# JMUWRobotics/3DTK

Hardware: AMD Instinct MI355X
Metric: NN correspondences/sec (1M-vs-1M pairwise ICP, full iteration) (higher is better)
Workload: dtype f64; 1 GPU; configs[1]: synthetic 1000000-vs-1000000 uniform pair, point-to-point ICP -a 1 -d 25 -b 20, 1xMI355X; points=1000000, bucket=20, minimizer=QUAT

## Files before the change

3dtk_amd/csrc/kernels.hip:

```cpp
#include <atomic>
#include <cstdio>
#include <vector>
#include <algorithm>
#include <hip/hip_runtime.h>
#include <type_traits>

#include <cmath>
#include <cstdio>
#include <cstdlib>
#include <cstring>

#include "kernels.h"
#include "lane_stack.h"
#ifdef TDTK_LAB
#include "loop_dev.h"
#endif

namespace tdtk {

#define WAVE 64
#define LAZY_MAX 8

__device__ __forceinline__ void dev_xf3(const Mat4& A, double x, double y, double z, double& ox,
                                        double& oy, double& oz)
// ... 125 lines not shown
  typedef uint32_t raw __attribute__((ext_vector_type(sizeof(V) / 4)));
  typedef const raw __attribute__((address_space(1))) * gp;
  const raw r = *(gp)(base + off);
  V v;
  __builtin_memcpy(&v, &r, sizeof v);
  return v;
}
template <class V>
__device__ __forceinline__ void gstore(char* base, const uint32_t off, const V v)
{
  typedef uint32_t raw __attribute__((ext_vector_type(sizeof(V) / 4)));
  typedef raw __attribute__((address_space(1))) * gp;
  raw r;
  __builtin_memcpy(&r, &v, sizeof v);
  *(gp)(base + off) = r;
}
#define TDTK_PIN_BATCH3(a, b, c) asm volatile("" : "+v"(a), "+v"(b), "+v"(c))

#define TDTK_PIN_V64(x) asm volatile("" : "+v"(x))
#define TDTK_PIN_S64(x) asm volatile("" : "+s"(x))
#define TDTK_PIN_S32(x) asm volatile("" : "+s"(x))
#define TDTK_PIN_SF(x) asm volatile("" : "+s"(x))
#define TDTK_PIN_VF(x) asm volatile("" : "+v"(x))

struct BoxF32 {
  float qx, qy, qz;
  float delta;
  float thi, tlo;
  float ec;
  float pthr;
  float qs, pthr16;
  __device__ __forceinline__ void set_query(const double x, const double y, const double z, const float absmax)
  {
    qx = (float)x; qy = (float)y; qz = (float)z;
    qs = 0.f;
    const float qm = fmaxf(fmaxf(fabsf(qx), fabsf(qy)), fabsf(qz));
    delta = 3.0e-7f * (qm + 2.0f * absmax) + 1.0e-30f;
    ec = 1.05e-7f * (qm + absmax) + 1.0e-30f;
    const float probe = fabsf(qx) + fabsf(qy) + fabsf(qz);
    if (!(probe <= 3.0e38f)) { delta = __builtin_nanf(""); ec = delta; }
  }
  __device__ __forceinline__ float reject_from(const float R) const
  {
    const float w = (R * 1.000001f + ec) * 1.000001f;
    const float t = w * w * 1.000001f;
    return (t <= 1.0e37f) ? t : __builtin_nanf("");
// ... 879 lines not shown
#pragma unroll
  for (int off = 32; off > 0; off >>= 1) t += __shfl_down(t, off, WAVE);
  return t;
}

template <int BLOCK, int SD, int GS = 8, bool FUSE = false, bool LOOP = false>
__global__ void __launch_bounds__(BLOCK) k_search_g8(const SearchArgs a_by_value)
{
  (void)a_by_value;
  search_g8_body<BLOCK, SD, GS, FUSE, LOOP>(kernarg_block<SearchArgs>(), blockIdx.x, gridDim.x);
}
template <int BLOCK, int SD, int GS>
__global__ void __launch_bounds__(BLOCK) k_search_g8_multi(const SearchArgs* __restrict__ args, const uint32_t* __restrict__ base,
                                                           int nbatch)
{
  int l = 0;
  while (l + 1 < nbatch && blockIdx.x >= base[l + 1]) ++l;
  l = __builtin_amdgcn_readfirstlane(l);
  const uint32_t b0 = base[l], b1 = base[l + 1];
  search_g8_body<BLOCK, SD, GS>(args[l], blockIdx.x - b0, b1 - b0);
}

#define WTRACE_MAX 32768u
#ifdef TDTK_LAB
__device__ unsigned long long g_wtrace[3 * WTRACE_MAX];
#else
__device__ unsigned long long g_wtrace[3];
#endif

struct RefillCfg {
  static constexpr int BLOCK = 128, SD = 4;
  static constexpr int THRESH = 16, WPS = 4;
  static constexpr bool COUNT = false;
  static constexpr int FUSE = 0;
  static constexpr bool ORDER = true; static constexpr int ORD_MAX = 256;
  static constexpr bool LAZY = false;
  static constexpr bool DEFER = false;
  static constexpr bool DYN = false, FAT = false, SHARE = false, PIPE = false;
  static constexpr int PTS = 4, PROBE = 0, TOP = 0;
};
template <class CFG>
__device__ __forceinline__ void search_refill_body(const SearchArgs& a, const uint32_t bid, const uint32_t nb)
{
  constexpr int BLOCK = CFG::BLOCK, SD = CFG::SD, THRESH = CFG::THRESH, FUSE = CFG::FUSE, PTS = CFG::PTS, PROBE = CFG::PROBE, ORD_MAX = CFG::ORD_MAX, TOP = CFG::TOP;
  constexpr bool COUNT = CFG::COUNT, DYN = CFG::DYN, ORDER = CFG::ORDER, FAT = CFG::FAT, LAZY = CFG::LAZY, SHARE = CFG::SHARE, PIPE = CFG::PIPE, DEFER = CFG::DEFER;
  __shared__ uint4 lds_stk[SD][BLOCK];
  __shared__ uint4 lds_top[TOP > 0 ? 3 * TOP : 1];
  uint32_t top_n = 0;
  if constexpr (TOP > 0) {
    top_n = min((uint32_t)TOP, a.T.n_hot);
    const uint4* __restrict__ h16 = reinterpret_cast<const uint4*>(a.T.hot);
    for (uint32_t k = threadIdx.x; k < 3u * top_n; k += BLOCK) lds_top[k] = h16[k];
    __syncthreads();
  }

  const size_t gl = (size_t)bid * BLOCK + threadIdx.x;
  const unsigned lane = threadIdx.x & (WAVE - 1);
  if (kLab && a.trace && lane == 0) {
    const uint32_t wid0 = bid * (BLOCK / WAVE) + threadIdx.x / WAVE;
    if (wid0 < WTRACE_MAX) g_wtrace[3 * wid0] = wall_clock64();
  }
  __shared__ double lds_mv[LAZY ? LAZY_MAX * 16 : 1];
  if constexpr (LAZY) {
    if (a.nmoves) {
      const double* gm = reinterpret_cast<const double*>(a.moves);
      for (int k = threadIdx.x; k < a.nmoves * 16; k += BLOCK) lds_mv[k] = gm[k];
      __syncthreads();
    }
  }
  LaneStackQ<BLOCK, SD> st;
  st.l_e = &lds_stk[0][threadIdx.x];
  st.g_m2 = a.ovf_m2; st.g_ref = a.ovf_ref; st.gcol = gl;
  st.gstride = (size_t)nb * BLOCK;
  st.sp = 0;

  const TreeDev& T = a.T;
  const double4* __restrict__ nodes = reinterpret_cast<const double4*>(T.nodes);
  const double4* __restrict__ pts = reinterpret_cast<const double4*>(T.pts);
  const LeafEntry* const t_leaf_tab = T.leaf_tab;
  const uint32_t t_cb = T.cb, t_cmask = T.cmask;
  int* const a_kpos = a.kpos;
  double* const a_d2 = a.d2;
  unsigned char* const a_cost = a.cost;
  const char* const t_grp = reinterpret_cast<const char*>(T.grp);
  const char* const t_fat = reinterpret_cast<const char*>(T.fat);
  typedef typename std::conditional<(ORD_MAX > 256), unsigned short, unsigned char>::type ord_t;
  __shared__ ord_t lds_order[ORDER ? BLOCK / WAVE : 1][ORDER ? ORD_MAX : 4];
  ord_t* const my_order = lds_order[ORDER ? threadIdx.x / WAVE : 0];
  constexpr bool CERT = DEFER && BUCKET_Q16 && !LAZY && !FAT && !PIPE && TOP == 0 && PROBE == 0 && FUSE == 3 && !DYN && !SHARE && ORDER;
  static_assert(!CERT || (ORD_MAX >= CERT_MAX_SLAB && ORD_MAX / WAVE <= 32), "a slab with certificates is one ordered piece");
  bool ordered = false;
  size_t piece0 = 0;
  uint32_t walkbits = 0xFFFFFFFFu, n_listed = 0;
  auto order_piece = [&](size_t p0, size_t p1) {
    ordered = false;
    piece0 = p0;
    if (!ORDER || !a.use_cost || !a.cost || p1 <= p0 || p1 - p0 > (size_t)ORD_MAX) return;
    const uint32_t cntp = (uint32_t)(p1 - p0);
    int cls[ORD_MAX / WAVE];
    unsigned cvv[ORD_MAX / WAVE];
    unsigned mn = 255u, mx = 0u;
#pragma unroll
    for (int r = 0; r < ORD_MAX / WAVE; r++) {
      const uint32_t o = (uint32_t)r * WAVE + lane;
      const bool w = o < cntp && (!CERT || ((walkbits >> r) & 1u) != 0u);
      cvv[r] = w ? (unsigned)a.cost[p0 + o] : 0u;
      if (w) { mn = min(mn, cvv[r]); mx = max(mx, cvv[r]); }
    }
#pragma unroll
    for (int off = 32; off > 0; off >>= 1) {
      mn = min(mn, (unsigned)__shfl_xor((int)mn, off, WAVE));
      mx = max(mx, (unsigned)__shfl_xor((int)mx, off, WAVE));
    }
    const unsigned span = (mx > mn) ? mx - mn + 1u : 1u;
#pragma unroll
    for (int r = 0; r < ORD_MAX / WAVE; r++) {
      const uint32_t o = (uint32_t)r * WAVE + lane;
      const bool w = o < cntp && (!CERT || ((walkbits >> r) & 1u) != 0u);
      cls[r] = w ? (int)min(((cvv[r] - mn) * 8u) / span, 7u) : -1;
    }
    uint32_t base = 0;
    for (int k = 7; k >= 0; k--) {
#pragma unroll
      for (int r = 0; r < ORD_MAX / WAVE; r++) {
        if ((uint32_t)r * WAVE >= cntp) continue;
        const unsigned long long m = __ballot(cls[r] == k);
        if (cls[r] == k) my_order[base + (uint32_t)__popcll(m & ((1ull << lane) - 1ull))] = (ord_t)(r * WAVE + lane);
        base += (uint32_t)__popcll(m);
      }
    }
    __builtin_amdgcn_fence(__ATOMIC_SEQ_CST, "wavefront");
    __builtin_amdgcn_wave_barrier();
    ordered = true;
    n_listed = base;
  };
  const bool certw = CERT && a.cert != nullptr;
  __shared__ uint4 lds_cert[CERT ? BLOCK : 1];
  float* const my_slot = reinterpret_cast<float*>(&lds_cert[CERT ? threadIdx.x : 0]);
  unsigned c_skh = 0, c_skn = 0, c_walk = 0;
  auto cert_sweep = [&](size_t p0, size_t p1) {
    walkbits = 0u;
    const uint32_t q0 = (uint32_t)p0, cntp = (uint32_t)(p1 - p0);
    for (uint32_t r = 0; r < (uint32_t)(ORD_MAX / WAVE); r++) {
      const uint32_t o = r * WAVE + lane;
      if (o >= cntp) continue;
      const uint32_t q = q0 + o, q8 = q << 3, q4 = q << 2;
      const SearchArgs* ap = &a;
      asm volatile("" : "+s"(ap));
      const int kp = gload<int>(reinterpret_cast<const char*>(a_kpos), q4);
      const float Lq = ap->cert_use ? gload<float>(reinterpret_cast<const char*>(ap->cert), q4) : 0.f;
      const double ox = gload<double>(reinterpret_cast<const char*>(ap->x), q8), oy = gload<double>(reinterpret_cast<const char*>(ap->y), q8),
                   oz = gload<double>(reinterpret_cast<const char*>(ap->z), q8);
      double tx = ox, ty = oy, tz = oz;
      if (ap->has_pending) {
        dev_xf3_inplace(ap->pending, tx, ty, tz);
        gstore<double>(reinterpret_cast<char*>(ap->x), q8, tx); gstore<double>(reinterpret_cast<char*>(ap->y), q8, ty);
        gstore<double>(reinterpret_cast<char*>(ap->z), q8, tz);
        if (ap->nx) {
          double px = ap->nx[q], py = ap->ny[q], pz = ap->nz[q];
          dev_xf3normal(ap->pending, px, py, pz);
          ap->nx[q] = px; ap->ny[q] = py; ap->nz[q] = pz;
        }
      }
      const SearchArgs* ap2 = &a;
      asm volatile("" : "+s"(ap2), "+v"(tx));
      double ax = ox, ay = oy, az = oz, bxq = tx, byq = ty, bzq = tz;
      if (ap2->has_inv) { dev_xf3(ap2->inv, ox, oy, oz, ax, ay, az); dev_xf3(ap2->inv, tx, ty, tz, bxq, byq, bzq); }
      const double ex = bxq - ax, ey = byq - ay, ez = bzq - az;
      const float mv = __builtin_amdgcn_sqrtf((float)(ex * ex + ey * ey + ez * ez) * 1.000001f) * 1.000001f;
      const float qm = fmaxf(fmaxf(fabsf((float)bxq), fabsf((float)byq)), fabsf((float)bzq));
      const SearchArgs* ap3 = &a;
      asm volatile("" : "+s"(ap3), "+v"(bxq));
      const double maxd2 = ap3->maxd2;
      const float R = __builtin_amdgcn_sqrtf((float)maxd2) * 1.000001f;
      const float eabs = 1.0e-9f * (ap3->T.absmax + R + qm) + 1.0e-30f;
      const float delta = mv + eabs;
      float dh = R;
      bool hit = false;
      if (kp >= 0) {
        const uint32_t po = (uint32_t)kp << 5;
        const double2 pxy = gload<double2>(reinterpret_cast<const char*>(pts), po);
        const double pzz = gload<double>(reinterpret_cast<const char*>(pts), po + 16);
        const double dx = pxy.x - bxq, dy = pxy.y - byq, dz = pzz - bzq;
        const double d = dx * dx + dy * dy + dz * dz;
        if (d < maxd2) { hit = true; dh = __builtin_amdgcn_sqrtf((float)d * 1.000001f) * 1.000001f; }
      }
      const float rhs = Lq - delta * 1.000001f - eabs;
      const bool skip = (kp >= 0) ? (hit && dh < rhs) : (dh <= rhs);
      const float mrg = fminf(fmaxf(ap3->cert_kappa * delta, ap3->cert_lo * dh), ap3->cert_hi * dh);
      if (!skip) walkbits |= 1u << r;
      gstore<float>(reinterpret_cast<char*>(ap3->cert), q4, skip ? rhs * 0.999999f : mrg);
      if (COUNT && skip) { if (kp >= 0) ++c_skh; else ++c_skn; }
    }
    __builtin_amdgcn_fence(__ATOMIC_SEQ_CST, "workgroup");
  };
  size_t next_q, end_q;
  __shared__ uint32_t lds_cursor;
  size_t wg0 = 0;
  uint32_t wg_len = 0;
  bool ord_on = false;
  size_t sub = 0, reg0 = 0, pstride = 0, slab_end = a.n;
  int nph = 1;
  bool exhausted = false;
  int phase = 0;
  uint32_t xq = 0, tried = 0, nslab = 0, per_x = 0;
  if (DYN) {
    next_q = end_q = 0;
    nslab = (uint32_t)((a.n + (size_t)a.slab - 1) / (size_t)a.slab);
    per_x = (nslab + 7u) >> 3;
    xq = (uint32_t)__builtin_amdgcn_s_getreg((3 << 11) | (0 << 6) | 20) & 7u;
    if (bid == 0 && threadIdx.x < 8) a.q_ctr_next[threadIdx.x] = 0u;
  } else {
    const uint32_t wpx = (nb >> 3) * (BLOCK / WAVE);
    const uint32_t wx = (uint32_t)__builtin_amdgcn_readfirstlane((int)((bid >> 3) * (BLOCK / WAVE) + threadIdx.x / WAVE));
    if (kLab && a.pool_slab) {
// ... 7 lines not shown
      if (bid == 0 && threadIdx.x < 8) a.q_ctr_next[threadIdx.x] = 0u;
    } else {
      if (kLab && !LAZY && a.bounds) {
        const uint32_t w = (bid & 7u) * wpx + wx;
        reg0 = (size_t)a.bounds[w];
        slab_end = (size_t)a.bounds[w + 1];
        if (slab_end > a.n) slab_end = a.n;
        if (reg0 > slab_end) reg0 = slab_end;
        sub = (size_t)ORD_MAX;
        pstride = sub;
        nph = (int)((slab_end - reg0 + sub - 1) / sub);
        if (nph < 1) nph = 1;
      } else {
        sub = (size_t)(a.qpw / a.phases);
        reg0 = (size_t)(bid & 7u) * wpx * (size_t)a.qpw + (size_t)wx * sub;
        pstride = (size_t)wpx * sub;
        slab_end = a.n;
        nph = a.phases;
      }
      next_q = reg0;
      end_q = next_q + sub;
      if (next_q > slab_end) next_q = slab_end;
      if (end_q > slab_end) end_q = slab_end;
      if (certw) cert_sweep(next_q, end_q);
      order_piece(next_q, end_q);
      if (certw && ordered) end_q = next_q + n_listed;
      walkbits = 0xFFFFFFFFu;
      if constexpr (SHARE) {
        wg0 = (size_t)(bid & 7u) * wpx * (size_t)a.qpw + (size_t)((bid >> 3) * (BLOCK / WAVE)) * sub;
        if (wg0 > a.n) wg0 = a.n;
        const size_t len = (size_t)(BLOCK / WAVE) * sub;
        wg_len = (uint32_t)((wg0 + len <= a.n) ? len : a.n - wg0);
        ord_on = ORDER && a.use_cost && a.cost && sub <= (size_t)ORD_MAX;
        if (threadIdx.x == 0) lds_cursor = 0u;
        __syncthreads();
      }
    }
  }

  if constexpr (LAZY && !DYN) {
    if (a.nmoves) {
      const uint32_t slab0 = (uint32_t)a.qpw, sub0 = (uint32_t)sub;
      const bool nrm = a.nx != nullptr;
      constexpr int MT = 5;
      for (uint32_t j0 = 0; j0 < slab0; j0 += MT * WAVE) {
        size_t q[MT];
        bool ok[MT];
        double px[MT], py[MT], pz[MT];
// ... 35 lines not shown
              ux = an; uy = bn; uz = cn;
            }
            a.nx[q[u]] = ux; a.ny[q[u]] = uy; a.nz[q[u]] = uz;
          }
        }
      }
      __builtin_amdgcn_fence(__ATOMIC_SEQ_CST, "workgroup");
    }
  }
  uint32_t cur = REF_DONE;
  double best = 0.0, qx = 0, qy = 0, qz = 0;
  int bk = -1;
  size_t qi = 0;
  bool have = false;
  BoxF32 bx;
  bx.qx = bx.qy = bx.qz = 0.f; bx.delta = 0.f; bx.thi = 0.f; bx.tlo = 0.f; bx.ec = 0.f; bx.pthr = 0.f; bx.qs = 0.f; bx.pthr16 = 0.f;
  constexpr bool USE_Q16 = BUCKET_Q16 && !LAZY;
  constexpr bool DEFER_OK = DEFER && USE_Q16 && !FAT && !PIPE && TOP == 0 && PROBE == 0;
  uint32_t q16xy = 0u, q16zz = 0u;
  bool q16in = false;
  const char* const t_q16 = USE_Q16 ? reinterpret_cast<const char*>(T.q16) : nullptr;
  auto q16_query = [&]() {
    if (USE_Q16 && (DEFER_OK || t_q16)) {
      const SearchArgs* ap = &a;
      asm volatile("" : "+s"(ap));
      bool out = false;
      const double sc = ap->T.q_scale;
      const uint32_t ix = (uint32_t)q16_index(qx, ap->T.q_lo[0], sc, out) & 0xFFFFu, iy = (uint32_t)q16_index(qy, ap->T.q_lo[1], sc, out) & 0xFFFFu,
                     iz = (uint32_t)q16_index(qz, ap->T.q_lo[2], sc, out) & 0xFFFFu;
      q16xy = ix | (iy << 16); q16zz = iz | (iz << 16); q16in = !out;
      bx.qs = (float)sc * 1.0000002f;
    }
  };
  const char* __restrict__ hotb = reinterpret_cast<const char*>(T.hot);
  const char* const splitb = DEFER_OK ? reinterpret_cast<const char*>(T.split) : nullptr;
  const uint32_t split_off = DEFER_OK ? (uint32_t)(splitb - hotb) : 0u;
  const double a_tie = DEFER_OK ? a.tie : 0.0;
  constexpr uint32_t NBK_DEFER = 0x80000000u, NBK_THIN = 0x40000000u, NBK_UCHK = 0x20000000u, NBK_COST = 0x1FFFFFFFu;
  constexpr bool DEFER_UCHK = false;
  constexpr uint32_t NBK_FIXW = NBK_UCHK;
  static_assert(!(CERT && DEFER_UCHK), "one bit");
  unsigned c_int = 0, c_leaf = 0, c_pts = 0, c_redo = 0;
  unsigned c_t1 = 0, c_t2 = 0;
  unsigned nbk = 0;
  constexpr int NACC = (FUSE == 2 || FUSE == 5) ? 18 : ACC_DD;
  double acc[NACC];
  if (FUSE) {
#pragma unroll
    for (int k = 0; k < NACC; k++) acc[k] = 0.0;
  }

  for (;;) {
    const bool idle = (cur == REF_DONE);
    if (idle && have) {
      if (CERT && (nbk & NBK_FIXW) != 0u) {
        const float sw = __builtin_amdgcn_sqrtf(f32_below(best)) * 0.999999f;
        const float dm = __builtin_amdgcn_sqrtf(f32_below(*reinterpret_cast<const double*>(my_slot))) * 0.999999f + my_slot[3];
        const float sr = __builtin_amdgcn_sqrtf(my_slot[2]) * 0.999999f;
        const float L = fminf(fminf(sw, dm), sr) * 0.999999f;
        const SearchArgs* ap = &a;
        asm volatile("" : "+s"(ap));
        gstore<float>(reinterpret_cast<char*>(ap->cert), (uint32_t)qi << 2, ((nbk & NBK_THIN) == 0u && sw >= 0.f && dm >= 0.f && sr >= 0.f && L > 0.f) ? L : 0.f);
      }
      if (DEFER_OK && (nbk & (NBK_DEFER | NBK_THIN)) == (NBK_DEFER | NBK_THIN)) {
        bk = -2; nbk = 255u;
      }
      gstore<int>(reinterpret_cast<char*>(a_kpos), (uint32_t)qi << 2, bk);
      if (ORDER && a_cost) a_cost[qi] = (unsigned char)min(nbk & NBK_COST, 255u);
      if (a_d2) gstore<double>(reinterpret_cast<char*>(a_d2), (uint32_t)qi << 3, best);
      have = false;
      if constexpr (FUSE == 2) if (bk >= 0) {
        const double tx = a.x[qi], ty = a.y[qi], tz = a.z[qi];
        const double4 c = *reinterpret_cast<const double4*>(reinterpret_cast<const char*>(pts) + ((uint32_t)bk << 5));
        double mx, my, mz;
        dev_xf3(a.A, c.x, c.y, c.z, mx, my, mz);
        const double dx = mx - tx, dy = my - ty, dz = mz - tz;
        const double x = (mx + tx) / 2.0, y = (my + ty) / 2.0, z = (mz + tz) / 2.0;
        acc[0] += 1.0;
        acc[1] += dx * dx + dy * dy + dz * dz;
        acc[2] += x; acc[3] += y; acc[4] += z;
        acc[5] += x * x + y * y;
        acc[6] += x * x + z * z;
        acc[7] += y * y + z * z;
        acc[8] += x * y; acc[9] += x * z; acc[10] += y * z;
        acc[11] += dx; acc[12] += dy; acc[13] += dz;
        acc[14] += -z * dy + y * dz;
        acc[15] += -y * dx + x * dy;
        acc[16] += z * dx - x * dz;
// ... 8 lines not shown
        acc[ACC_N] += 1.0;
        acc[ACC_SUM] += px * px + py * py + pz * pz;
        const double m0 = mx - a.shift[0], m1 = my - a.shift[1], m2 = mz - a.shift[2];
        const double d0 = tx - a.shift[0], d1 = ty - a.shift[1], d2 = tz - a.shift[2];
        acc[ACC_SM + 0] += m0; acc[ACC_SM + 1] += m1; acc[ACC_SM + 2] += m2;
        acc[ACC_SD + 0] += d0; acc[ACC_SD + 1] += d1; acc[ACC_SD + 2] += d2;
        acc[ACC_P + 0] += m0 * d0; acc[ACC_P + 1] += m0 * d1; acc[ACC_P + 2] += m0 * d2;
        acc[ACC_P + 3] += m1 * d0; acc[ACC_P + 4] += m1 * d1; acc[ACC_P + 5] += m1 * d2;
        acc[ACC_P + 6] += m2 * d0; acc[ACC_P + 7] += m2 * d1; acc[ACC_P + 8] += m2 * d2;
      }
    }
    const unsigned long long idlem = __ballot(idle);
    const unsigned long long activem = __ballot(!idle);
    const bool fill = (activem == 0 || __popcll(idlem) >= THRESH);
#ifdef TDTK_LAB
#include "lab_draws.inc"
#endif
    if (!DYN && !a.pool_slab && fill && next_q >= end_q && phase + 1 < nph) {
      ++phase;
      next_q = reg0 + (size_t)phase * pstride;
      end_q = next_q + sub;
      if (next_q > slab_end) next_q = slab_end;
      if (end_q > slab_end) end_q = slab_end;
      order_piece(next_q, end_q);
    }
    uint32_t sh_base = 0;
    bool sh_draw = false;
    if constexpr (SHARE) {
      if (fill && !exhausted) {
        if (lane == 0) sh_base = atomicAdd(&lds_cursor, (uint32_t)__popcll(idlem));
        sh_base = (uint32_t)__builtin_amdgcn_readfirstlane((int)sh_base);
        if (sh_base >= wg_len) exhausted = true; else sh_draw = true;
      }
    }
    if (SHARE ? sh_draw : (next_q < end_q && fill)) {
      const unsigned rank = (unsigned)__popcll(idlem & ((1ull << lane) - 1ull));
      size_t slot, mine;
      bool got;
      if constexpr (SHARE) {
        const uint32_t pos = sh_base + rank;
        got = idle && pos < wg_len;
        const uint32_t pj = pos / (uint32_t)sub, po = pos - pj * (uint32_t)sub;
        slot = wg0 + pos;
        mine = (ord_on && got) ? wg0 + (size_t)pj * sub + (size_t)lds_order[ORDER ? pj : 0][po] : slot;
      } else {
        slot = next_q + rank;
        got = idle && slot < end_q;
        mine = (ORDER && got && ordered) ? piece0 + (size_t)my_order[slot - piece0] : slot;
      }
      if (PIPE && got) {
        bk = a.warm ? gload<int>(reinterpret_cast<const char*>(a_kpos), (uint32_t)mine << 2) : -1;
        const uint32_t m8 = (uint32_t)mine << 3;
        qx = gload<double>(reinterpret_cast<const char*>(a.x), m8); qy = gload<double>(reinterpret_cast<const char*>(a.y), m8);
        qz = gload<double>(reinterpret_cast<const char*>(a.z), m8);
        qi = mine; have = true; nbk = 0; st.sp = 0;
        cur = REF_STAGE1;
      }
      if (!PIPE && got) {
        const uint32_t m8 = (uint32_t)mine << 3;
        const SearchArgs* hp = &a;
        bool certh = false;
        if constexpr (CERT) {
          asm volatile("" : "+s"(hp));
          certh = hp->cert != nullptr;
        }
        const int kp_prev = a.warm ? gload<int>(reinterpret_cast<const char*>(a_kpos), (uint32_t)mine << 2) : -1;
        double tx = gload<double>(reinterpret_cast<const char*>(a.x), m8), ty = gload<double>(reinterpret_cast<const char*>(a.y), m8),
               tz = gload<double>(reinterpret_cast<const char*>(a.z), m8);
        if (a.has_pending && !certh) {
          dev_xf3_inplace(a.pending, tx, ty, tz);
          gstore<double>(reinterpret_cast<char*>(a.x), m8, tx); gstore<double>(reinterpret_cast<char*>(a.y), m8, ty);
          gstore<double>(reinterpret_cast<char*>(a.z), m8, tz);
          if (a.nx) {
            double px = a.nx[mine], py = a.ny[mine], pz = a.nz[mine];
            dev_xf3normal(a.pending, px, py, pz);
            a.nx[mine] = px; a.ny[mine] = py; a.nz[mine] = pz;
          }
        }
        if (a.skip && a.skip[mine]) {
          gstore<int>(reinterpret_cast<char*>(a_kpos), (uint32_t)mine << 2, -1);
          if (ORDER && a_cost) a_cost[mine] = 0;
          if (a_d2) gstore<double>(reinterpret_cast<char*>(a_d2), m8, a.maxd2);
        } else {
        qx = tx; qy = ty; qz = tz;
        if (a.has_inv) dev_xf3(a.inv, tx, ty, tz, qx, qy, qz);
        qi = mine; have = true; nbk = 0;
        cur = T.root_ref; best = warm_radius_kp(a, kp_prev, qx, qy, qz); bk = -1; st.sp = 0;
        if (DEFER_OK) nbk = (DEFER_UCHK && !(kp_prev >= 0 && best < a.maxd2)) ? (NBK_DEFER | NBK_UCHK) : NBK_DEFER;
        if (COUNT) ++c_walk;
        if (certh) {
          float m = gload<float>(reinterpret_cast<const char*>(hp->cert), (uint32_t)mine << 2);
          if (!(m >= 0.f)) m = 0.f;
          nbk |= NBK_FIXW;
          *reinterpret_cast<double*>(my_slot) = best; my_slot[2] = __builtin_inff(); my_slot[3] = m;
          const double rw = (double)(__builtin_amdgcn_sqrtf((float)best) * 1.000001f + m);
          const double W = rw * rw;
          if (W >= best) best = W;
        }
        bx.set_query(qx, qy, qz, T.absmax);
        q16_query();
        bx.set_radius(best);
        }
      }
      next_q += (size_t)__popcll(idlem);
    }
    if (__ballot(cur != REF_DONE) == 0) {
      if constexpr (SHARE) { if (exhausted) break; continue; }
      if (next_q >= end_q && (DYN ? tried >= 8u : ((kLab && a.pool_slab) ? exhausted : phase + 1 >= nph))) break;
      continue;
    }

#ifdef TDTK_LAB
#include "lab_fat_walk.inc"
#endif
    if constexpr (!FAT) while (!(cur & REF_LEAF) || (PIPE && cur == REF_STAGE1)) {
      double w_x = 0.0, w_y = 0.0, w_z = 0.0;
      bool fin = false;
#ifdef TDTK_LAB
#include "lab_pipe_stage.inc"
#endif
      if (!PIPE || !(cur & REF_LEAF)) {
      if (COUNT) ++c_int;
      if (COUNT && kLab) { const unsigned long long on = __ballot(true); if ((int)lane == __ffsll((long long)on) - 1) ++c_t1; }
      if (ORDER) ++nbk;
      bool need_pop = false;
      uint32_t next = REF_DONE;
      const uint32_t ucur = __builtin_amdgcn_readfirstlane(cur);
// ... 143 lines not shown
          for (int j = 0; j < PTS; j++) {
            const bool take = dd[j] < cd, again = j > 0 && oo[j] == oo[j - 1];
            if (take && cd - dd[j] <= a_tie) nbk |= NBK_THIN;
            ru = (take ? bk >= 0 : !again) ? fminf(ru, f32_below(take ? cd : dd[j])) : ru;
            if (take) { cd = dd[j]; bk = (int)(oo[j] >> 5); }
          }
        }
      }
      if constexpr (CERT) {
        if (fixw) { *reinterpret_cast<double*>(my_slot) = cd; my_slot[2] = ru; }
        else best = cd;
      }
      }
      if (!fixw) bx.set_radius(best);
      cur = REF_DONE;
      while (st.sp > 0) {
        --st.sp;
        uint32_t r; double m2;
        st.top(r, m2);
        if (fixw || m2 < best) { cur = r; break; }
      }
    }
  }
  if constexpr (DEFER_OK) {
    __builtin_amdgcn_fence(__ATOMIC_SEQ_CST, "workgroup");
    const SearchArgs* ap = &a;
    asm volatile("" : "+s"(ap));
    const bool balanced = kLab && ap->bounds != nullptr;
    const uint32_t slab = balanced ? (uint32_t)(slab_end - reg0) : (uint32_t)ap->qpw, sub32 = balanced ? 0x7FFFFFFFu : (uint32_t)sub;
    for (uint32_t j0 = 0; j0 < slab; j0 += WAVE) {
      uint32_t j = j0 + lane, ph = 0;
      const bool in = j < slab;
      while (j >= sub32 && in) { j -= sub32; ph++; }
      const size_t q = reg0 + (size_t)ph * pstride + j;
      if (!(in && q < slab_end)) continue;
      if (gload<int>(reinterpret_cast<const char*>(a_kpos), (uint32_t)q << 2) != -2) continue;
      if (COUNT) ++c_redo;
      const uint32_t q8 = (uint32_t)q << 3;
      const double tx = gload<double>(reinterpret_cast<const char*>(ap->x), q8), ty = gload<double>(reinterpret_cast<const char*>(ap->y), q8),
                   tz = gload<double>(reinterpret_cast<const char*>(ap->z), q8);
      double rx = tx, ry = ty, rz = tz;
      if (ap->has_inv) dev_xf3(ap->inv, tx, ty, tz, rx, ry, rz);
      double rbest = ap->maxd2;
      int rbk = -1;
      unsigned r_int = 0, r_leaf = 0, r_pts = 0;
      kd_search_plain(reinterpret_cast<const char*>(ap->T.nodes), reinterpret_cast<const char*>(ap->T.pts), t_leaf_tab, t_cb, t_cmask,
                      ap->T.root_ref, rx, ry, rz, rbest, rbk, st, r_int, r_leaf, r_pts);
      if (COUNT) { c_int += r_int; c_leaf += r_leaf; c_pts += r_pts; }
      gstore<int>(reinterpret_cast<char*>(a_kpos), (uint32_t)q << 2, rbk);
      if (ORDER && a_cost) a_cost[q] = (unsigned char)min(r_int + 4u * r_leaf, 255u);
      if (a_d2) gstore<double>(reinterpret_cast<char*>(a_d2), q8, rbest);
    }
  }
  if (kLab && a.trace && lane == 0) {
    const uint32_t wid = bid * (BLOCK / WAVE) + threadIdx.x / WAVE;
    if (wid < WTRACE_MAX) {
      g_wtrace[3 * wid + 1] = wall_clock64();
      g_wtrace[3 * wid + 2] = (unsigned long long)(__builtin_amdgcn_s_getreg((3 << 11) | (0 << 6) | 20) & 7u) |
                              ((unsigned long long)(unsigned)__builtin_amdgcn_s_getreg((31 << 11) | (0 << 6) | 4) << 8);
    }
  }
  if (COUNT && a.counters) {
    const unsigned long long s_int = wave_sum_u(c_int), s_leaf = wave_sum_u(c_leaf), s_pts = wave_sum_u(c_pts);
    if (lane == 0) {
      atomicAdd(&a.counters[0], s_int);
      atomicAdd(&a.counters[1], s_leaf);
      atomicAdd(&a.counters[2], s_pts);
    }
    if (DEFER_OK) {
      const unsigned long long s_redo = wave_sum_u(c_redo);
      if (lane == 0 && s_redo) atomicAdd(&a.counters[7], s_redo);
    }
    {
      const unsigned long long s_skh = wave_sum_u(c_skh), s_skn = wave_sum_u(c_skn), s_walk = wave_sum_u(c_walk);
      if (lane == 0) {
        if (s_skh) atomicAdd(&a.counters[10], s_skh);
        if (s_skn) atomicAdd(&a.counters[11], s_skn);
        if (s_walk) atomicAdd(&a.counters[12], s_walk);
      }
    }
    if (kLab) {
// ... 45 lines not shown
            acc[7] += y * y + z * z;
            acc[8] += x * y; acc[9] += x * z; acc[10] += y * z;
            acc[11] += dx; acc[12] += dy; acc[13] += dz;
            acc[14] += -z * dy + y * dz;
            acc[15] += -y * dx + x * dy;
            acc[16] += z * dx - x * dz;
            acc[17] += x * dx + y * dy + z * dz;
            continue;
          }
          const double px = mx - tx[u], py = my - ty[u], pz = mz - tz[u];
          acc[ACC_N] += 1.0;
          acc[ACC_SUM] += px * px + py * py + pz * pz;
          const double m0 = mx - a.shift[0], m1 = my - a.shift[1], m2 = mz - a.shift[2];
          const double d0 = tx[u] - a.shift[0], d1 = ty[u] - a.shift[1], d2 = tz[u] - a.shift[2];
          acc[ACC_SM + 0] += m0; acc[ACC_SM + 1] += m1; acc[ACC_SM + 2] += m2;
          acc[ACC_SD + 0] += d0; acc[ACC_SD + 1] += d1; acc[ACC_SD + 2] += d2;
          acc[ACC_P + 0] += m0 * d0; acc[ACC_P + 1] += m0 * d1; acc[ACC_P + 2] += m0 * d2;
          acc[ACC_P + 3] += m1 * d0; acc[ACC_P + 4] += m1 * d1; acc[ACC_P + 5] += m1 * d2;
          acc[ACC_P + 6] += m2 * d0; acc[ACC_P + 7] += m2 * d1; acc[ACC_P + 8] += m2 * d2;
        }
      }
    }
  }
  if (FUSE) {
    constexpr int NW = BLOCK / WAVE;
    __shared__ double red[NW][NACC];
    const int wv = threadIdx.x / WAVE;
#pragma unroll
    for (int k = 0; k < NACC; k++) {
      const double s = wave_sum(acc[k]);
      if (lane == 0) red[wv][k] = s;
    }
    __syncthreads();
    constexpr int RS = (BLOCK > 128) ? BLOCK / 128 : 1, WPR = NW / RS;
    for (int kk = threadIdx.x; kk < RS * ACC_TOTAL; kk += BLOCK) {
      const int sr = kk / ACC_TOTAL, k = kk - sr * ACC_TOTAL;
      int src = -1;
      if (FUSE == 2 || FUSE == 5) src = (k == ACC_N) ? 0 : (k == ACC_SUM) ? 1 : (k >= ACC_L && k < ACC_L + 15) ? 2 + (k - ACC_L) : (k == ACC_LU) ? 17 : -1;
      else if (k < ACC_DD) src = k;
      double s = 0.0;
      if (src >= 0)
        for (int w = 0; w < WPR; w++) s += red[sr * WPR + w][src];
      const size_t row = (RS == 1) ? (size_t)bid : ((size_t)((bid >> 3) * RS + sr) * 8u + (bid & 7u));
      a.partials[row * ACC_TOTAL + k] = s;
    }
  }
// ... 558 lines not shown
#ifdef TDTK_LAB
  if (const size_t lanes = lab_max_lanes(n)) return lanes;
#endif
  int q;
  const size_t a = (size_t)search_grid(n) * SEARCH_BLOCK;
  const size_t b = std::max((size_t)refill_grid_b(n, 128, &q) * 128, (size_t)refill_grid_b(n, 64, &q) * 64);
  const size_t c = (size_t)refill_grid_b(n, SEARCH_BLOCK, &q) * SEARCH_BLOCK;
  const size_t d = (size_t)num_cu() * 4 * 8 * WAVE;
  return std::max(std::max(a, b), std::max(c, d));
}
uint32_t search_fused_rows(size_t n, int side_by_side)
{
  const int v = pick_variant(n);
  if (v == 10) return g8_grid4(n);
  if (v == 4) return search_grid(n);
#ifdef TDTK_LAB
  if (const uint32_t rows = lab_fused_rows(n, side_by_side)) return rows;
#endif
  int q;
  return refill_grid_b(n, 128, &q, side_by_side);
}
bool search_cert_capable(const SearchArgs& a)
{
  if (kLab || !BUCKET_Q16 || pick_variant(a.n) != 20 || a.fuse != 3) return false;
  if (!(a.warm && a.tie > 0.0 && a.T.split != nullptr && a.T.q16 != nullptr)) return false;
  if (!(a.use_cost && a.cost != nullptr) || a.skip != nullptr || a.d2 != nullptr || a.side_by_side > 1) return false;
  int qpw;
  (void)refill_grid_b(a.n, 128, &qpw, a.side_by_side);
  return qpw <= CERT_MAX_SLAB;
}
template <bool COUNT, int FUSE>
static void launch_refill128(SearchArgs& a, hipStream_t s)
{
  if (a.cert && !(FUSE == 3 && search_cert_capable(a))) a.cert = nullptr;
#ifdef TDTK_LAB
  if (lab_refill_own_grid<COUNT, FUSE>(a, s)) return;
#endif
  int qpw;
  const uint32_t nb = refill_grid_b(a.n, 128, &qpw, a.side_by_side);
  a.qpw = qpw;
  {
    static std::atomic<int> launches{0};
    static const int want = [] { const char* e = lab_env("TDTK_WAVE_TRACE"); return e ? atoi(e) : -1; }();
    a.trace = (want >= 0 && launches.fetch_add(1) == want) ? 1 : 0;
  }
  a.pool_slab = 0; a.region = 0;
  const int pool_pct = (FUSE == 3) ? 0 : refill_pool_pct(a.n, a.side_by_side);
  if (pool_pct > 0) {
    const size_t R = (((a.n + 7) / 8) + 63) & ~(size_t)63;
    const size_t wpx = (size_t)(nb >> 3) * 2;
    size_t qs = (R * (size_t)(100 - pool_pct) / 100 / wpx) & ~(size_t)31;
    if (qs < 64) qs = 64;
    a.qpw = (int)qs; a.region = R;
    const char* e = lab_env("TDTK_REFILL_POOL_SLAB");
    a.pool_slab = e ? std::max(16, atoi(e)) : 64;
  }
  int ph = ((a.n + 255) / 256 >= (size_t)num_cu() * 4 * 7 || a.side_by_side > 1 || a.pool_slab) ? 1 : 2;
  if (a.use_cost) ph = 1;
  if (FUSE == 3) ph = 1;
  if (const char* e = lab_env("TDTK_REFILL_PHASES")) ph = atoi(e);
  if (ph < 1) ph = 1;
  while (ph > 1 && (qpw % (ph * 16)) != 0) --ph;
  a.phases = ph;
  static const unsigned occ_lds = [] { const char* e = lab_env("TDTK_OCC_LDS"); return e ? (unsigned)atoi(e) : 0u; }();
  bool launched = false;
#ifdef TDTK_LAB
  launched = lab_refill_on_grid<COUNT, FUSE>(a, nb, occ_lds, s);
#endif
  if constexpr (FUSE == 0 || FUSE == 3) {
    const bool defer = a.warm && a.tie > 0.0 && a.T.split != nullptr && a.T.q16 != nullptr && BUCKET_Q16 && !a.pool_slab;
    const bool thresh32 = refill_thresh(a.n) == 32;
    if (launched) {}
    else if (thresh32 && defer) launch_refill<SinglePass<32, COUNT, FUSE, true>>(nb, occ_lds, s, a);
    else if (thresh32) launch_refill<SinglePass<32, COUNT, FUSE, false>>(nb, occ_lds, s, a);
    else if (defer) launch_refill<SinglePass<16, COUNT, FUSE, true>>(nb, occ_lds, s, a);
    else launch_refill<SinglePass<16, COUNT, FUSE, false>>(nb, occ_lds, s, a);
  }
  if (kLab && a.trace) {
    (void)hipStreamSynchronize(s);
    const uint32_t nw = std::min<uint32_t>(nb * 2u, WTRACE_MAX);
    std::vector<unsigned long long> h(3 * (size_t)nw);
    if (hipMemcpyFromSymbol(h.data(), HIP_SYMBOL(g_wtrace), h.size() * sizeof(unsigned long long)) == hipSuccess)
      for (uint32_t w = 0; w < nw; w++)
        fprintf(stderr, "WTRACE %u %u %llu %llu %llu\n", w / 2u, w % 2u, h[3 * w + 2], h[3 * w], h[3 * w + 1]);
  }
}

hipError_t launch_search(const SearchArgs& a_in, uint32_t grid, int dirmode, bool count, hipStream_t s)
{
  if (a_in.n == 0) return hipSuccess;
  SearchArgs a = a_in;
  {
    const char* e = lab_env("TDTK_FAT_SMALL");
    if (!(e && e[0] == '1') && pick_variant(a.n) != 20) a.T.fat = nullptr;
  }
  if (!kLab) { a.bounds = nullptr; a.trace = 0; }
  dim3 g(grid), b(SEARCH_BLOCK);
  if (dirmode == 1) hipLaunchKernelGGL((k_search<SEARCH_BLOCK, 8, false, 1, false, 1>), g, b, 0, s, a);
  else if (dirmode == 2) hipLaunchKernelGGL((k_search<SEARCH_BLOCK, 8, false, 2, false, 1>), g, b, 0, s, a);
  else {
    int v = pick_variant(a.n);
    if (a.skip && !(v == 20 || v == 4 || v == 10)) v = (a.n >= (size_t)262144) ? 20 : ((a.n >= (size_t)98304) ? 4 : 10);
    if (a.fuse && !(v == 20 || ((v == 10 || v == 4) && !count))) return hipErrorInvalidValue;
    if (!kLab && v == 20 && !(a.fuse == 0 || a.fuse == 3)) return hipErrorInvalidValue;
#ifdef TDTK_LAB
    hipError_t lab_err;
    if (lab_launch_search(a, v, count, g, s, &lab_err)) return lab_err;
// ... 388 lines not shown
```

Before: 15.41 billion NN correspondences/s.

## Batch cert-sweep loads, hoist normal transforms, and skip redo pass for thin-free waves

Restructures the certificate sweep so all rows' kpos, cert, coordinate, cost and hit-point loads are issued up front in batches. The per-row serial loads are replaced by a fully unrolled compute loop, and the normal-vector transform becomes a separate batched pass. The sweep's preloaded cost values are reused when ordering, so the cost bytes are not read twice. Each wave also records in LDS whether any query was marked thin, and skips the deferred redo slab loop when none were. Matrices and arguments are read through constant address-space pointers. Wave-trace instrumentation is extended as well. Register pressure rises from holding several rows of doubles live at once.

```diff
diff --git a/3dtk_amd/csrc/kernels.hip b/3dtk_amd/csrc/kernels.hip
--- a/3dtk_amd/csrc/kernels.hip
+++ b/3dtk_amd/csrc/kernels.hip
@@ -171,6 +171,7 @@
 #define TDTK_PIN_S32(x) asm volatile("" : "+s"(x))
 #define TDTK_PIN_SF(x) asm volatile("" : "+s"(x))
 #define TDTK_PIN_VF(x) asm volatile("" : "+v"(x))
+#define TDTK_PIN_V32(x) asm volatile("" : "+v"(x))
 
 struct BoxF32 {
   float qx, qy, qz;
@@ -1096,10 +1097,11 @@
 }
 
 #define WTRACE_MAX 32768u
+enum { WT_ENTRY = 0, WT_REDO = 1, WT_HWID = 2, WT_SWEEP = 3, WT_ORDER = 4, WT_FIRST = 5, WT_LOOP = 6, WT_SUMS = 7, WT_WORDS = 8 };
 #ifdef TDTK_LAB
-__device__ unsigned long long g_wtrace[3 * WTRACE_MAX];
+__device__ unsigned long long g_wtrace[WT_WORDS * WTRACE_MAX];
 #else
-__device__ unsigned long long g_wtrace[3];
+__device__ unsigned long long g_wtrace[WT_WORDS];
 #endif
 
 struct RefillCfg {
@@ -1113,6 +1115,22 @@
   static constexpr bool DYN = false, FAT = false, SHARE = false, PIPE = false;
   static constexpr int PTS = 4, PROBE = 0, TOP = 0;
 };
+typedef const SearchArgs __attribute__((address_space(4))) * args_kp;
+typedef const Mat4 __attribute__((address_space(4))) * mat_kp;
+__device__ __forceinline__ args_kp args_here(const SearchArgs& a)
+{
+  args_kp p = (args_kp)&a;
+  asm volatile("" : "+s"(p));
+  return p;
+}
+__device__ __forceinline__ Mat4 mat_here(const mat_kp m)
+{
+  Mat4 A;
+#pragma unroll
+  for (int k = 0; k < 16; k++) A.m[k] = ((k & 3) == 3) ? 0.0 : m->m[k];
+  return A;
+}
+
 template <class CFG>
 __device__ __forceinline__ void search_refill_body(const SearchArgs& a, const uint32_t bid, const uint32_t nb)
 {
@@ -1132,8 +1150,14 @@
   const unsigned lane = threadIdx.x & (WAVE - 1);
   if (kLab && a.trace && lane == 0) {
     const uint32_t wid0 = bid * (BLOCK / WAVE) + threadIdx.x / WAVE;
-    if (wid0 < WTRACE_MAX) g_wtrace[3 * wid0] = wall_clock64();
-  }
+    if (wid0 < WTRACE_MAX) { g_wtrace[WT_WORDS * wid0 + WT_FIRST] = 0ull; g_wtrace[WT_WORDS * wid0 + WT_ENTRY] = wall_clock64(); }
+  }
+  auto wtrace_at = [&](const int word) {
+    if (kLab && a.trace && lane == 0) {
+      const uint32_t wid0 = bid * (BLOCK / WAVE) + threadIdx.x / WAVE;
+      if (wid0 < WTRACE_MAX) g_wtrace[WT_WORDS * wid0 + word] = wall_clock64();
+    }
+  };
   __shared__ double lds_mv[LAZY ? LAZY_MAX * 16 : 1];
   if constexpr (LAZY) {
     if (a.nmoves) {
@@ -1166,7 +1190,7 @@
   bool ordered = false;
   size_t piece0 = 0;
   uint32_t walkbits = 0xFFFFFFFFu, n_listed = 0;
-  auto order_piece = [&](size_t p0, size_t p1) {
+  auto order_piece = [&](size_t p0, size_t p1, const unsigned* pre) {
     ordered = false;
     piece0 = p0;
     if (!ORDER || !a.use_cost || !a.cost || p1 <= p0 || p1 - p0 > (size_t)ORD_MAX) return;
@@ -1178,7 +1202,7 @@
     for (int r = 0; r < ORD_MAX / WAVE; r++) {
       const uint32_t o = (uint32_t)r * WAVE + lane;
       const bool w = o < cntp && (!CERT || ((walkbits >> r) & 1u) != 0u);
-      cvv[r] = w ? (unsigned)a.cost[p0 + o] : 0u;
+      cvv[r] = w ? (pre ? pre[r] : (unsigned)a.cost[p0 + o]) : 0u;
       if (w) { mn = min(mn, cvv[r]); mx = max(mx, cvv[r]); }
     }
 #pragma unroll
@@ -1212,59 +1236,137 @@
   __shared__ uint4 lds_cert[CERT ? BLOCK : 1];
   float* const my_slot = reinterpret_cast<float*>(&lds_cert[CERT ? threadIdx.x : 0]);
   unsigned c_skh = 0, c_skn = 0, c_walk = 0;
+  unsigned sw_cost[ORD_MAX / WAVE];
   auto cert_sweep = [&](size_t p0, size_t p1) {
+    constexpr int NR = ORD_MAX / WAVE;
     walkbits = 0u;
     const uint32_t q0 = (uint32_t)p0, cntp = (uint32_t)(p1 - p0);
-    for (uint32_t r = 0; r < (uint32_t)(ORD_MAX / WAVE); r++) {
-      const uint32_t o = r * WAVE + lane;
-      if (o >= cntp) continue;
+    int kp[NR];
+    float Lq[NR];
+    double ox[NR], oy[NR], oz[NR], hz[NR];
+    double2 hxy[NR];
+    if (cntp == 0u) return;
+    {
+      const args_kp ap = args_here(a);
+      const char* const gx = reinterpret_cast<const char*>(ap->x);
+      const char* const gy = reinterpret_cast<const char*>(ap->y);
+      const char* const gz = reinterpret_cast<const char*>(ap->z);
+      const char* const gc = reinterpret_cast<const char*>(ap->cert);
+      const bool use = ap->cert_use != 0;
+      const char* const gk = (ap->use_cost && a_cost) ? reinterpret_cast<const char*>(a_cost) : nullptr;
+      uint32_t qc[NR];
+#pragma unroll
+      for (int r = 0; r < NR; r++) {
+        qc[r] = q0 + min((uint32_t)r * WAVE + lane, cntp - 1u);
+        kp[r] = gload<int>(reinterpret_cast<const char*>(a_kpos), qc[r] << 2);
+      }
+#pragma unroll
+      for (int r = 0; r < NR; r++) {
+        Lq[r] = gload<float>(gc, qc[r] << 2);
+        ox[r] = gload<double>(gx, qc[r] << 3); oy[r] = gload<double>(gy, qc[r] << 3); oz[r] = gload<double>(gz, qc[r] << 3);
+      }
+#pragma unroll
+      for (int r = 0; r < NR; r++) sw_cost[r] = 0u;
+      if (gk) {
+#pragma unroll
+        for (int r = 0; r < NR; r++) sw_cost[r] = (unsigned)*(const unsigned char __attribute__((address_space(1)))*)(gk + qc[r]);
+      }
+#pragma unroll
+      for (int r = 0; r < NR; r++) TDTK_PIN_V32(kp[r]);
+#pragma unroll
+      for (int r = 0; r < NR; r++) { hxy[r] = make_double2(0.0, 0.0); hz[r] = 0.0; }
+      if (ap->T.n_slots != 0u) {
+#pragma unroll
+        for (int r = 0; r < NR; r++) {
+          const uint32_t po = (kp[r] >= 0) ? (uint32_t)kp[r] << 5 : 0u;
+          hxy[r] = gload<double2>(reinterpret_cast<const char*>(pts), po);
+          hz[r] = gload<double>(reinterpret_cast<const char*>(pts), po + 16);
+        }
+      }
+#pragma unroll
+      for (int r = 0; r < NR; r++) {
+        TDTK_PIN_BATCH3(ox[r], oy[r], oz[r]);
+        TDTK_PIN_BATCH3(hxy[r].x, hxy[r].y, hz[r]);
+        TDTK_PIN_VF(Lq[r]);
+        TDTK_PIN_V32(sw_cost[r]);
+        if (!use) Lq[r] = 0.f;
+      }
+    }
+#pragma unroll
+    for (int r = 0; r < NR; r++) {
+      const uint32_t o = (uint32_t)r * WAVE + lane;
+      if ((uint32_t)r * WAVE >= cntp) continue;
+      const bool in = o < cntp;
       const uint32_t q = q0 + o, q8 = q << 3, q4 = q << 2;
-      const SearchArgs* ap = &a;
-      asm volatile("" : "+s"(ap));
-      const int kp = gload<int>(reinterpret_cast<const char*>(a_kpos), q4);
-      const float Lq = ap->cert_use ? gload<float>(reinterpret_cast<const char*>(ap->cert), q4) : 0.f;
-      const double ox = gload<double>(reinterpret_cast<const char*>(ap->x), q8), oy = gload<double>(reinterpret_cast<const char*>(ap->y), q8),
-                   oz = gload<double>(reinterpret_cast<const char*>(ap->z), q8);
-      double tx = ox, ty = oy, tz = oz;
+      double tx = ox[r], ty = oy[r], tz = oz[r];
+      const args_kp ap = args_here(a);
       if (ap->has_pending) {
-        dev_xf3_inplace(ap->pending, tx, ty, tz);
-        gstore<double>(reinterpret_cast<char*>(ap->x), q8, tx); gstore<double>(reinterpret_cast<char*>(ap->y), q8, ty);
-        gstore<double>(reinterpret_cast<char*>(ap->z), q8, tz);
-        if (ap->nx) {
-          double px = ap->nx[q], py = ap->ny[q], pz = ap->nz[q];
-          dev_xf3normal(ap->pending, px, py, pz);
-          ap->nx[q] = px; ap->ny[q] = py; ap->nz[q] = pz;
-        }
-      }
-      const SearchArgs* ap2 = &a;
-      asm volatile("" : "+s"(ap2), "+v"(tx));
-      double ax = ox, ay = oy, az = oz, bxq = tx, byq = ty, bzq = tz;
-      if (ap2->has_inv) { dev_xf3(ap2->inv, ox, oy, oz, ax, ay, az); dev_xf3(ap2->inv, tx, ty, tz, bxq, byq, bzq); }
+        const Mat4 P = mat_here(&ap->pending);
+        dev_xf3_inplace(P, tx, ty, tz);
+        if (in) {
+          gstore<double>(reinterpret_cast<char*>(ap->x), q8, tx); gstore<double>(reinterpret_cast<char*>(ap->y), q8, ty);
+          gstore<double>(reinterpret_cast<char*>(ap->z), q8, tz);
+        }
+      }
+      const args_kp ap2 = args_here(a);
+      TDTK_PIN_V64(tx);
+      double ax = ox[r], ay = oy[r], az = oz[r], bxq = tx, byq = ty, bzq = tz;
+      if (ap2->has_inv) {
+        const Mat4 I = mat_here(&ap2->inv);
+        dev_xf3(I, ox[r], oy[r], oz[r], ax, ay, az); dev_xf3(I, tx, ty, tz, bxq, byq, bzq);
+      }
       const double ex = bxq - ax, ey = byq - ay, ez = bzq - az;
       const float mv = __builtin_amdgcn_sqrtf((float)(ex * ex + ey * ey + ez * ez) * 1.000001f) * 1.000001f;
       const float qm = fmaxf(fmaxf(fabsf((float)bxq), fabsf((float)byq)), fabsf((float)bzq));
-      const SearchArgs* ap3 = &a;
-      asm volatile("" : "+s"(ap3), "+v"(bxq));
+      const args_kp ap3 = args_here(a);
+      TDTK_PIN_V64(bxq);
       const double maxd2 = ap3->maxd2;
       const float R = __builtin_amdgcn_sqrtf((float)maxd2) * 1.000001f;
       const float eabs = 1.0e-9f * (ap3->T.absmax + R + qm) + 1.0e-30f;
       const float delta = mv + eabs;
       float dh = R;
       bool hit = false;
-      if (kp >= 0) {
-        const uint32_t po = (uint32_t)kp << 5;
-        const double2 pxy = gload<double2>(reinterpret_cast<const char*>(pts), po);
-        const double pzz = gload<double>(reinterpret_cast<const char*>(pts), po + 16);
-        const double dx = pxy.x - bxq, dy = pxy.y - byq, dz = pzz - bzq;
+      if (kp[r] >= 0) {
+        const double dx = hxy[r].x - bxq, dy = hxy[r].y - byq, dz = hz[r] - bzq;
         const double d = dx * dx + dy * dy + dz * dz;
         if (d < maxd2) { hit = true; dh = __builtin_amdgcn_sqrtf((float)d * 1.000001f) * 1.000001f; }
       }
-      const float rhs = Lq - delta * 1.000001f - eabs;
-      const bool skip = (kp >= 0) ? (hit && dh < rhs) : (dh <= rhs);
+      const float rhs = Lq[r] - delta * 1.000001f - eabs;
+      const bool skip = (kp[r] >= 0) ? (hit && dh < rhs) : (dh <= rhs);
       const float mrg = fminf(fmaxf(ap3->cert_kappa * delta, ap3->cert_lo * dh), ap3->cert_hi * dh);
-      if (!skip) walkbits |= 1u << r;
-      gstore<float>(reinterpret_cast<char*>(ap3->cert), q4, skip ? rhs * 0.999999f : mrg);
-      if (COUNT && skip) { if (kp >= 0) ++c_skh; else ++c_skn; }
+      if (in) {
+        if (!skip) walkbits |= 1u << r;
+        gstore<float>(reinterpret_cast<char*>(ap3->cert), q4, skip ? rhs * 0.999999f : mrg);
+        if (COUNT && skip) { if (kp[r] >= 0) ++c_skh; else ++c_skn; }
+      }
+    }
+    {
+      const args_kp ap = args_here(a);
+      if (ap->has_pending && ap->nx) {
+        double* const gnx = ap->nx; double* const gny = ap->ny; double* const gnz = ap->nz;
+        const Mat4 P = mat_here(&ap->pending);
+        double ux[NR], uy[NR], uz[NR];
+#pragma unroll
+        for (int r = 0; r < NR; r++) {
+          const uint32_t o = (uint32_t)r * WAVE + lane, q8 = (q0 + o) << 3;
+          ux[r] = uy[r] = uz[r] = 0.0;
+          if (o < cntp) {
+            ux[r] = gload<double>(reinterpret_cast<const char*>(gnx), q8); uy[r] = gload<double>(reinterpret_cast<const char*>(gny), q8);
+            uz[r] = gload<double>(reinterpret_cast<const char*>(gnz), q8);
+          }
+        }
+#pragma unroll
+        for (int r = 0; r < NR; r++) TDTK_PIN_BATCH3(ux[r], uy[r], uz[r]);
+#pragma unroll
+        for (int r = 0; r < NR; r++) {
+          const uint32_t o = (uint32_t)r * WAVE + lane, q8 = (q0 + o) << 3;
+          dev_xf3normal(P, ux[r], uy[r], uz[r]);
+          if (o < cntp) {
+            gstore<double>(reinterpret_cast<char*>(gnx), q8, ux[r]); gstore<double>(reinterpret_cast<char*>(gny), q8, uy[r]);
+            gstore<double>(reinterpret_cast<char*>(gnz), q8, uz[r]);
+          }
+        }
+      }
     }
     __builtin_amdgcn_fence(__ATOMIC_SEQ_CST, "workgroup");
   };
@@ -1318,8 +1420,9 @@
       end_q = next_q + sub;
       if (next_q > slab_end) next_q = slab_end;
       if (end_q > slab_end) end_q = slab_end;
-      if (certw) cert_sweep(next_q, end_q);
-      order_piece(next_q, end_q);
+      if (certw) { cert_sweep(next_q, end_q); wtrace_at(WT_SWEEP); order_piece(next_q, end_q, sw_cost); }
+      else { wtrace_at(WT_SWEEP); order_piece(next_q, end_q, nullptr); }
+      wtrace_at(WT_ORDER);
       if (certw && ordered) end_q = next_q + n_listed;
       walkbits = 0xFFFFFFFFu;
       if constexpr (SHARE) {
@@ -1401,8 +1504,7 @@
   const char* const t_q16 = USE_Q16 ? reinterpret_cast<const char*>(T.q16) : nullptr;
   auto q16_query = [&]() {
     if (USE_Q16 && (DEFER_OK || t_q16)) {
-      const SearchArgs* ap = &a;
-      asm volatile("" : "+s"(ap));
+      const args_kp ap = args_here(a);
       bool out = false;
       const double sc = ap->T.q_scale;
       const uint32_t ix = (uint32_t)q16_index(qx, ap->T.q_lo[0], sc, out) & 0xFFFFu, iy = (uint32_t)q16_index(qy, ap->T.q_lo[1], sc, out) & 0xFFFFu,
@@ -1415,6 +1517,8 @@
   const char* const splitb = DEFER_OK ? reinterpret_cast<const char*>(T.split) : nullptr;
   const uint32_t split_off = DEFER_OK ? (uint32_t)(splitb - hotb) : 0u;
   const double a_tie = DEFER_OK ? a.tie : 0.0;
+  __shared__ uint32_t lds_thin[DEFER_OK ? BLOCK / WAVE : 1];
+  if (DEFER_OK && lane == 0) lds_thin[threadIdx.x / WAVE] = 0u;
   constexpr uint32_t NBK_DEFER = 0x80000000u, NBK_THIN = 0x40000000u, NBK_UCHK = 0x20000000u, NBK_COST = 0x1FFFFFFFu;
   constexpr bool DEFER_UCHK = false;
   constexpr uint32_t NBK_FIXW = NBK_UCHK;
@@ -1437,12 +1541,12 @@
         const float dm = __builtin_amdgcn_sqrtf(f32_below(*reinterpret_cast<const double*>(my_slot))) * 0.999999f + my_slot[3];
         const float sr = __builtin_amdgcn_sqrtf(my_slot[2]) * 0.999999f;
         const float L = fminf(fminf(sw, dm), sr) * 0.999999f;
-        const SearchArgs* ap = &a;
-        asm volatile("" : "+s"(ap));
+        const args_kp ap = args_here(a);
         gstore<float>(reinterpret_cast<char*>(ap->cert), (uint32_t)qi << 2, ((nbk & NBK_THIN) == 0u && sw >= 0.f && dm >= 0.f && sr >= 0.f && L > 0.f) ? L : 0.f);
       }
       if (DEFER_OK && (nbk & (NBK_DEFER | NBK_THIN)) == (NBK_DEFER | NBK_THIN)) {
         bk = -2; nbk = 255u;
+        lds_thin[threadIdx.x / WAVE] = 1u;
       }
       gstore<int>(reinterpret_cast<char*>(a_kpos), (uint32_t)qi << 2, bk);
       if (ORDER && a_cost) a_cost[qi] = (unsigned char)min(nbk & NBK_COST, 255u);
@@ -1497,7 +1601,7 @@
       end_q = next_q + sub;
       if (next_q > slab_end) next_q = slab_end;
       if (end_q > slab_end) end_q = slab_end;
-      order_piece(next_q, end_q);
+      order_piece(next_q, end_q, nullptr);
     }
     uint32_t sh_base = 0;
     bool sh_draw = false;
@@ -1533,12 +1637,9 @@
       }
       if (!PIPE && got) {
         const uint32_t m8 = (uint32_t)mine << 3;
-        const SearchArgs* hp = &a;
-        bool certh = false;
-        if constexpr (CERT) {
-          asm volatile("" : "+s"(hp));
-          certh = hp->cert != nullptr;
-        }
+        const char* h_cert = nullptr;
+        if constexpr (CERT) h_cert = reinterpret_cast<const char*>(args_here(a)->cert);
+        const bool certh = h_cert != nullptr;
         const int kp_prev = a.warm ? gload<int>(reinterpret_cast<const char*>(a_kpos), (uint32_t)mine << 2) : -1;
         double tx = gload<double>(reinterpret_cast<const char*>(a.x), m8), ty = gload<double>(reinterpret_cast<const char*>(a.y), m8),
                tz = gload<double>(reinterpret_cast<const char*>(a.z), m8);
@@ -1564,7 +1665,7 @@
         if (DEFER_OK) nbk = (DEFER_UCHK && !(kp_prev >= 0 && best < a.maxd2)) ? (NBK_DEFER | NBK_UCHK) : NBK_DEFER;
         if (COUNT) ++c_walk;
         if (certh) {
-          float m = gload<float>(reinterpret_cast<const char*>(hp->cert), (uint32_t)mine << 2);
+          float m = gload<float>(h_cert, (uint32_t)mine << 2);
           if (!(m >= 0.f)) m = 0.f;
           nbk |= NBK_FIXW;
           *reinterpret_cast<double*>(my_slot) = best; my_slot[2] = __builtin_inff(); my_slot[3] = m;
@@ -1578,6 +1679,13 @@
         }
       }
       next_q += (size_t)__popcll(idlem);
+      if (kLab && a.trace) {
+        TDTK_PIN_V64(best);
+        if (lane == 0) {
+          const uint32_t wid0 = bid * (BLOCK / WAVE) + threadIdx.x / WAVE;
+          if (wid0 < WTRACE_MAX && g_wtrace[WT_WORDS * wid0 + WT_FIRST] == 0ull) g_wtrace[WT_WORDS * wid0 + WT_FIRST] = wall_clock64();
+        }
+      }
     }
     if (__ballot(cur != REF_DONE) == 0) {
       if constexpr (SHARE) { if (exhausted) break; continue; }
@@ -1767,12 +1875,15 @@
       }
     }
   }
+  wtrace_at(WT_LOOP);
   if constexpr (DEFER_OK) {
     __builtin_amdgcn_fence(__ATOMIC_SEQ_CST, "workgroup");
-    const SearchArgs* ap = &a;
-    asm volatile("" : "+s"(ap));
+    const args_kp ap = args_here(a);
     const bool balanced = kLab && ap->bounds != nullptr;
-    const uint32_t slab = balanced ? (uint32_t)(slab_end - reg0) : (uint32_t)ap->qpw, sub32 = balanced ? 0x7FFFFFFFu : (uint32_t)sub;
+    uint32_t slab = balanced ? (uint32_t)(slab_end - reg0) : (uint32_t)ap->qpw;
+    const uint32_t sub32 = balanced ? 0x7FFFFFFFu : (uint32_t)sub;
+    if (!SHARE && !DYN && !(kLab && ap->pool_slab) &&
+        __builtin_amdgcn_readfirstlane((int)lds_thin[threadIdx.x / WAVE]) == 0) slab = 0u;
     for (uint32_t j0 = 0; j0 < slab; j0 += WAVE) {
       uint32_t j = j0 + lane, ph = 0;
       const bool in = j < slab;
@@ -1785,7 +1896,7 @@
       const double tx = gload<double>(reinterpret_cast<const char*>(ap->x), q8), ty = gload<double>(reinterpret_cast<const char*>(ap->y), q8),
                    tz = gload<double>(reinterpret_cast<const char*>(ap->z), q8);
       double rx = tx, ry = ty, rz = tz;
-      if (ap->has_inv) dev_xf3(ap->inv, tx, ty, tz, rx, ry, rz);
+      if (ap->has_inv) { const Mat4 I = mat_here(&ap->inv); dev_xf3(I, tx, ty, tz, rx, ry, rz); }
       double rbest = ap->maxd2;
       int rbk = -1;
       unsigned r_int = 0, r_leaf = 0, r_pts = 0;
@@ -1800,8 +1911,8 @@
   if (kLab && a.trace && lane == 0) {
     const uint32_t wid = bid * (BLOCK / WAVE) + threadIdx.x / WAVE;
     if (wid < WTRACE_MAX) {
-      g_wtrace[3 * wid + 1] = wall_clock64();
-      g_wtrace[3 * wid + 2] = (unsigned long long)(__builtin_amdgcn_s_getreg((3 << 11) | (0 << 6) | 20) & 7u) |
+      g_wtrace[WT_WORDS * wid + WT_REDO] = wall_clock64();
+      g_wtrace[WT_WORDS * wid + WT_HWID] = (unsigned long long)(__builtin_amdgcn_s_getreg((3 << 11) | (0 << 6) | 20) & 7u) |
                               ((unsigned long long)(unsigned)__builtin_amdgcn_s_getreg((31 << 11) | (0 << 6) | 4) << 8);
     }
   }
@@ -1893,6 +2004,8 @@
       }
     }
   }
+  if (kLab && FUSE) TDTK_PIN_V64(acc[0]);
+  wtrace_at(WT_SUMS);
   if (FUSE) {
     constexpr int NW = BLOCK / WAVE;
     __shared__ double red[NW][NACC];
@@ -2497,7 +2610,7 @@
 }
 bool search_cert_capable(const SearchArgs& a)
 {
-  if (kLab || !BUCKET_Q16 || pick_variant(a.n) != 20 || a.fuse != 3) return false;
+  if ((kLab && !lab_env("TDTK_WAVE_TRACE")) || !BUCKET_Q16 || pick_variant(a.n) != 20 || a.fuse != 3) return false;
   if (!(a.warm && a.tie > 0.0 && a.T.split != nullptr && a.T.q16 != nullptr)) return false;
   if (!(a.use_cost && a.cost != nullptr) || a.skip != nullptr || a.d2 != nullptr || a.side_by_side > 1) return false;
   int qpw;
@@ -2514,10 +2627,19 @@
   int qpw;
   const uint32_t nb = refill_grid_b(a.n, 128, &qpw, a.side_by_side);
   a.qpw = qpw;
+  int trace_idx = -1;
   {
     static std::atomic<int> launches{0};
-    static const int want = [] { const char* e = lab_env("TDTK_WAVE_TRACE"); return e ? atoi(e) : -1; }();
-    a.trace = (want >= 0 && launches.fetch_add(1) == want) ? 1 : 0;
+    static const std::vector<int> want = [] {
+      std::vector<int> w;
+      for (const char* e = lab_env("TDTK_WAVE_TRACE"); e && *e; ) { w.push_back(atoi(e)); e = strchr(e, ','); if (e) ++e; }
+      return w;
+    }();
+    a.trace = 0;
+    if (!want.empty()) {
+      trace_idx = launches.fetch_add(1);
+      a.trace = std::find(want.begin(), want.end(), trace_idx) != want.end() ? 1 : 0;
+    }
   }
   a.pool_slab = 0; a.region = 0;
   const int pool_pct = (FUSE == 3) ? 0 : refill_pool_pct(a.n, a.side_by_side);
@@ -2554,10 +2676,15 @@
   if (kLab && a.trace) {
     (void)hipStreamSynchronize(s);
     const uint32_t nw = std::min<uint32_t>(nb * 2u, WTRACE_MAX);
-    std::vector<unsigned long long> h(3 * (size_t)nw);
-    if (hipMemcpyFromSymbol(h.data(), HIP_SYMBOL(g_wtrace), h.size() * sizeof(unsigned long long)) == hipSuccess)
-      for (uint32_t w = 0; w < nw; w++)
-        fprintf(stderr, "WTRACE %u %u %llu %llu %llu\n", w / 2u, w % 2u, h[3 * w + 2], h[3 * w], h[3 * w + 1]);
+    std::vector<unsigned long long> h(WT_WORDS * (size_t)nw);
+    if (hipMemcpyFromSymbol(h.data(), HIP_SYMBOL(g_wtrace), h.size() * sizeof(unsigned long long)) == hipSuccess) {
+      fprintf(stderr, "WTRACE_LAUNCH %d n %zu cert %d cert_use %d warm %d qpw %d\n", trace_idx, a.n, a.cert ? 1 : 0, a.cert ? a.cert_use : 0, a.warm, a.qpw);
+      for (uint32_t w = 0; w < nw; w++) {
+        const unsigned long long* t = &h[WT_WORDS * (size_t)w];
+        fprintf(stderr, "WTRACE %u %u %llu %llu %llu %llu %llu %llu %llu %llu\n", w / 2u, w % 2u, t[WT_HWID], t[WT_ENTRY], t[WT_REDO], t[WT_SWEEP],
+                t[WT_ORDER], t[WT_FIRST], t[WT_LOOP], t[WT_SUMS]);
+      }
+    }
   }
 }
 
```

Result: faster. 18.71 billion NN correspondences/s (median of 6 runs) (+21.4%).
